# adam-kerrigan/pybader

Measured on AMD Instinct MI355X. Metric: Mvoxels/s neargrid assign+refine on 512^3 grid, higher is better.
Workload: dtype f64; 1 GPU; 512^3 synthetic 8-Gaussian-atom cubic cell (BASELINE config 3), neargrid assign + neargrid edge refinement changed:2, density resident in HBM; method=neargrid, device_driven_slab_step=False, basins=8

## Files before the change

### pybader_amd/csrc/host_assign.h

```cpp

static int read_counter(xb_ctx *c, int idx, int *out);
static GridL light(const Grid &g);

enum { BB_TOTAL = 1 << 20, BB_REGMAX = 1 << 16, BB_REGFIRST = 1 << 17 };

static bool table_windowed(const xb_ctx *c) { return c->g.wlen < c->g.nx; }

static int ensure_brick_bytes(xb_ctx *c, int nbr) {
    if (c->blab_alloc < nbr) {
        hipFree(c->blab_buf); c->blab_buf = nullptr; c->blab_alloc = 0; c->brick_rec = nullptr; c->brick_max_valid = false;
        if (c->grad_cover) { c->grad_cover = 0; c->grad_valid = false; }
        HIPCHK(hipMalloc(&c->blab_buf, (size_t)nbr * sizeof(int) + (size_t)nbr + 16));
        c->blab_alloc = nbr;
        c->brick_rec = reinterpret_cast<unsigned char *>(c->blab_buf + nbr);
    }
    return XB_OK;
}

static int ensure_grad(xb_ctx *c, bool force, bool boxes, bool main_rule) {
    if (int rc = need_grad(c)) return rc;
    c->g.main_ties = main_rule ? 1 : 0;
    if (c->grad_valid && !force && (c->grad_rule == 2 || c->grad_rule == (main_rule ? 1 : 0))) return XB_OK;
    const Grid &g = c->g;
    if (c->grad_valid && !force && !boxes && c->grad_cover == 1 && c->brick_rec) {
// ... 467 lines not shown
        else {
            k_buni_after_relabel<<<(nbr + 255) / 256, 256, 0, c->stream>>>(nbr, c->blab, box_max, c->first, buni, fs + FS_SORT_OK, nullptr, nullptr, nullptr);
            k_label_uniform_list<<<2048, TPB, 0, c->stream>>>(gl, c->labels, nb1, nb2, walk, 0, fs + FS_N_WALK, fs + FS_SORT_OK, buni);
        }
    } else
        k_relabel<<<nblocks(c->N), TPB, 0, c->stream>>>(g, c->labels, c->first, fs + FS_SORT_OK);
    k_reset_first<<<8, 256, 0, c->stream>>>(c->first, c->max_aux, 0, fs + FS_N_MAX, fs + FS_SORT_OK);
    HIPCHK(hipGetLastError());
    return XB_OK;
}

static int assign_neargrid_fused(xb_ctx *c, int64_t *n_maxima) {
    if (int rc = need_grad(c)) return rc;
    Grid &g = c->g;
    const GridL gl0 = light(g);
    const int nb0 = (g.nx + BRK - 1) / BRK, nb1 = (g.ny + BRK - 1) / BRK, nb2 = (g.nz + BRK - 1) / BRK, nbr = nb0 * nb1 * nb2;
    const bool part = g.nx % BRK || g.ny % BRK || g.nz % BRK;
    if (int rc = ensure_brick_bytes(c, nbr)) return rc;
    int *fs = c->fs;
    int *seed = c->list, *bmask = c->list + nbr, *buf0 = c->list + 2 * nbr, *buf1 = c->list + 3 * nbr, *walk = c->list + 4 * nbr;
    int *box_max = c->boxbuf + BB_REGMAX, *box_first = c->boxbuf + BB_REGFIRST;
    int *bmaxv = walk;
    int *bpot = c->list + 5 * nbr;
    const bool chase = true;
    int *bres = nullptr;
    c->box_max_tab = box_max;
    auto stage_done = [&](const char *what) {
        if (c->opt_dbg & 32) {
            const hipError_t e = (hipStreamSynchronize)(c->stream);
            int h16[16] = {0};
            (void)hipMemcpy(h16, fs, sizeof h16, hipMemcpyDeviceToHost);
            fprintf(stderr, "[assign] %s: %s  seeds %d regions %d certain %d walk %d maxima %d ovf %d err %d\n", what, hipGetErrorString(e), h16[FS_N_SEEDS],
                    h16[FS_N_BOXES], h16[FS_N_CERTAIN], h16[FS_N_WALK], h16[FS_N_MAX], h16[FS_N_OVF], h16[FS_ERR]);
            fflush(stderr);
        }
    };
    HIPCHK(hipMemsetAsync(fs, 0, FS_TOTAL * sizeof(int), c->stream));
    if (!c->first_clean) {
        k_fill<int><<<4096, TPB, 0, c->stream>>>(c->first, XB_INT_MAX, c->N);
        HIPCHK(hipGetLastError());
    }
    c->first_clean = false;
    c->regions_pending = false;
    c->buni_valid = false; c->regions_labels = false;
    c->list_valid = false; c->chg_n = -1;
    g.main_ties = 1;
    const GridL gl = light(g);
    (void)gl0;
    {
        ScopedTimer t4(c, 4);
        {
            ScopedTimer t5(c, 5);
            const int small = (g.nx < 16 || g.ny < 16 || g.nz < 80);
            dim3 grid((g.nz + GT_Z - 1) / GT_Z, (g.ny + GT_Y - 1) / GT_Y, (g.nx + GT_X - 1) / GT_X);
            GridS gs;
            const bool sym = sym_grid(g, gs);
            {
                int mirror = 0;
                double mu_scale = 0.;
                if (sym && c->opt_mirror) mirror_prefilter(g, mirror, mu_scale);
                const bool diag = c->opt_mask_diag && g.T[1] == 0. && g.T[2] == 0. && g.T[3] == 0. && g.T[5] == 0. && g.T[6] == 0. && g.T[7] == 0.;
                if (part) {
                    if (sym && diag) k_brick_masks<GridS, 1, true, true><<<grid, TPB, 0, c->stream>>>(gs, c->rho, small, bmask, bmaxv, fs + FS_TIES, 0, mu_scale, mirror, bpot);
                    else if (sym) k_brick_masks<GridS, 1, false, true><<<grid, TPB, 0, c->stream>>>(gs, c->rho, small, bmask, bmaxv, fs + FS_TIES, 0, mu_scale, mirror, bpot);
                    else k_brick_masks<Grid, 1, false, true><<<grid, TPB, 0, c->stream>>>(g, c->rho, small, bmask, bmaxv, fs + FS_TIES, 0, 0., 0, bpot);
                } else
                if (sym && diag) k_brick_masks<GridS, 1, true><<<grid, TPB, 0, c->stream>>>(gs, c->rho, small, bmask, bmaxv, fs + FS_TIES, 0, mu_scale, mirror, bpot);
                else if (sym) k_brick_masks<GridS, 1, false><<<grid, TPB, 0, c->stream>>>(gs, c->rho, small, bmask, bmaxv, fs + FS_TIES, 0, mu_scale, mirror, bpot);
                else k_brick_masks<Grid, 1, false><<<grid, TPB, 0, c->stream>>>(g, c->rho, small, bmask, bmaxv, fs + FS_TIES, 0, 0., 0, bpot);
            }
        }
        stage_done("brick masks");
        c->grad_valid = true;
        c->grad_rule = 1;
        c->grad_cover = 1;
        {
            k_seed_bricks<<<(nbr + 255) / 256, 256, 0, c->stream>>>(nbr, bmask, bmaxv, fs, seed, buf0, box_max, box_first);
            if (chase) {
                k_grow_parent<<<(nbr + TPB - 1) / TPB, TPB, 0, c->stream>>>(nb0, nb1, nb2, bmask, bpot, seed, buf1);
                k_grow_chase<<<(nbr + TPB - 1) / TPB, TPB, 0, c->stream>>>(nbr, buf1, seed, buf0, 4 * (nb0 + nb1 + nb2) + 64, fs);
            } else
                k_seed_finish<<<1, 1, 0, c->stream>>>(fs);
        }
        const int long_schedule = 2 * ((std::max(std::max(nb0, nb1), nb2) + BG - 1) / BG) + 12;
        const int launches = chase ? std::min(long_schedule, c->grow_kill_launches) : long_schedule;
        const dim3 ggrid((nb2 + BG - 1) / BG, (nb1 + BG - 1) / BG, (nb0 + BG - 1) / BG);
        for (int l = 0; l < launches; l++)
            k_brick_grow_dev<<<ggrid, BG * BG * BG, 0, c->stream>>>(nb0, nb1, nb2, bmask, seed, buf0, buf1, fs, BG, 0);
        k_grow_finish<<<64, TPB, 0, c->stream>>>(nbr, seed, buf0, buf1, fs, c->blab_buf, box_first, bmask, c->brick_rec, 0, chase && launches < long_schedule ? 1 : 0);
        HIPCHK(hipGetLastError());
        stage_done("region growth");
    }
    c->blab = c->blab_buf;
    c->regions_neargrid = true;
    c->walk = walk;
    c->nbk[0] = nb0; c->nbk[1] = nb1; c->nbk[2] = nb2;
    const long long own = c->N;
    {
        ScopedTimer t0(c, 0);
        {
            int bits = 0;
            while ((1 << bits) < std::max(std::max(nb0, nb1), nb2)) bits++;
            const unsigned n_codes = 1u << (3 * bits);
            const bool vac = c->has_vacuum && c->vac_by_tol;
            k_brick_walk_list_morton<<<(n_codes + 16 * TPB - 1) / (16 * TPB), TPB, 0, c->stream>>>(nb0, nb1, nb2, n_codes, c->blab, walk,
                                                                                                  fs + FS_N_WALK, fs + FS_GROW_RETRY,
                                                                                                  vac ? bpot : nullptr, c->vac_tol);
        }
        {
            ScopedTimer t7(c, 7);
            const int small = (g.nx < 16 || g.ny < 16 || g.nz < 80);
            GridS gs;
            if (sym_grid(g, gs))
                k_brick_records<GridS><<<4096, TPB, 0, c->stream>>>(gs, c->rho, c->grad, walk, fs + FS_N_WALK, nbr, nb1, nb2, c->brick_rec, small);
            else
                k_brick_records<Grid><<<4096, TPB, 0, c->stream>>>(g, c->rho, c->grad, walk, fs + FS_N_WALK, nbr, nb1, nb2, c->brick_rec, small);
        }
        stage_done("walk list + records");
        if (c->has_vacuum)
            k_fill_certain<<<nblocks(own), TPB, 0, c->stream>>>(gl, c->blab, nb1, nb2, box_max, c->labels, c->first, c->max_list,
                                                                fs + FS_N_MAX, c->max_cap, fs + FS_GROW_RETRY);
        else {
// ... 309 lines not shown
```

### pybader_amd/csrc/host_slab_table.h

```cpp


int xb_set_table_window(xb_ctx *c, int64_t margin) {
    NEED_GRID("xb_set_table_window");
    Grid &g = c->g;
    c->grad_valid = false;
    c->table_stage = 0;
    const int own = g.x1 - g.x0;
    if (margin < 0 || own == g.nx) { g.wx0 = 0; g.wlen = g.nx; c->table_margin = -1; g.wbase = 0; return XB_OK; }
    if (g.nx % 8 || g.ny % 8 || g.nz % 8 || g.x0 % 8 || g.x1 % 8)
        return fail(XB_E_ARG, "xb_set_table_window: grid and slab must be made of whole 8^3 bricks");
    const int m8 = (int)((std::max<int64_t>(margin, c->halo) + 7) / 8) * 8;
    if (own + 2 * m8 >= g.nx) { g.wx0 = 0; g.wlen = g.nx; c->table_margin = -1; g.wbase = 0; return XB_OK; }
    g.wx0 = ((g.x0 - m8) % g.nx + g.nx) % g.nx;
    g.wlen = own + 2 * m8;
    c->table_margin = m8;
    return need_grad(c);
}
static bool slab_sparse_ok(const xb_ctx *c) {
    const Grid &g = c->g;
    return c->opt_boxes && c->opt_bricks && table_windowed(c) && g.nx % BRK == 0 && g.ny % BRK == 0 && g.nz % BRK == 0 &&
           g.x0 % BRK == 0 && g.x1 % BRK == 0 && g.ny >= 16 && g.nz >= 16 && 7LL * (c->N / (BRK * BRK * BRK)) <= c->N;
}
int xb_table_build(xb_ctx *c, int64_t *n_local_seeds) {
    NEED_GRID_RAW("xb_table_build");
    if (int rc = need_grad(c)) return rc;
    c->slab_sparse = false;
    if (slab_sparse_ok(c)) {
        Grid &g = c->g;
        const int nb1 = g.ny / BRK, nb2 = g.nz / BRK, nbr = (g.nx / BRK) * nb1 * nb2;
        if (int rc = ensure_brick_bytes(c, nbr)) return rc;
        int *fs = c->fs, *bmask = c->list + nbr, *bmaxv = c->list + 4 * nbr;
        HIPCHK(hipMemsetAsync(fs, 0, FS_TOTAL * sizeof(int), c->stream));
        g.main_ties = 1;
        {
            ScopedTimer t4(c, 4);
            ScopedTimer t5(c, 5);
            const int small = (g.nx < 16 || g.ny < 16 || g.nz < 80);
            dim3 grid((g.nz + GT_Z - 1) / GT_Z, (g.ny + GT_Y - 1) / GT_Y, (g.x1 - g.x0) / GT_X);
            GridS gs;
            int mirror = 0;
            double mu_scale = 0.;
            if (c->opt_mirror) mirror_prefilter(g, mirror, mu_scale);
            if (sym_grid(g, gs)) k_brick_masks<GridS, 1, false><<<grid, TPB, 0, c->stream>>>(gs, c->rho, small, bmask, bmaxv, fs + FS_TIES, g.x0, mu_scale, mirror, nullptr);
            else k_brick_masks<Grid, 1, false><<<grid, TPB, 0, c->stream>>>(g, c->rho, small, bmask, bmaxv, fs + FS_TIES, g.x0, 0., 0, nullptr);
        }
        HIPCHK(hipGetLastError());
        int ties = 0;
        HIPCHK(hipMemcpyAsync(c->host_ints, fs + FS_TIES, sizeof(int), hipMemcpyDeviceToHost, c->stream));
        HIPCHK(hipStreamSynchronize(c->stream));
        ties = c->host_ints[0];
        c->window_ties = ties != 0;
        c->window_seeds.clear();
        c->grad_valid = true;
        c->grad_cover = 1;
        c->grad_rule = 1;
        c->blab = nullptr;
        c->n_boxes = 0; c->box_voxels = 0;
        c->table_stage = 1;
        c->slab_sparse = true;
        if (n_local_seeds) *n_local_seeds = 0;
        return XB_OK;
    }
    if (int rc = ensure_grad(c, true, true, true)) return rc;
    if (n_local_seeds) *n_local_seeds = table_windowed(c) ? (int64_t)c->window_seeds.size() : 0;
    return XB_OK;
}
int xb_table_local_seeds(xb_ctx *c, int64_t *out, int64_t capacity) {
    NEED_GRID_RAW("xb_table_local_seeds");
    if ((int64_t)c->window_seeds.size() > capacity) return fail(XB_E_ARG, "xb_table_local_seeds: capacity too small");
    for (size_t i = 0; i < c->window_seeds.size(); i++) out[i] = c->window_seeds[i];
    return XB_OK;
}
int xb_brick_masks(xb_ctx *c, void **dev_ptr, int64_t *n_bricks, int64_t *own_first, int64_t *own_count) {
    NEED_GRID_RAW("xb_brick_masks");
    const Grid &g = c->g;
    if (g.nx % 8 || g.ny % 8 || g.nz % 8) return fail(XB_E_STATE, "xb_brick_masks: grid is not made of whole bricks");
    const int64_t nbr = c->N / 512, per_plane = (int64_t)(g.ny / 8) * (g.nz / 8);
    if (dev_ptr) *dev_ptr = (void *)(c->list + nbr);
    if (n_bricks) *n_bricks = nbr;
    if (own_first) *own_first = (g.x0 / 8) * per_plane;
    if (own_count) *own_count = ((g.x1 - g.x0) / 8) * per_plane;
    return XB_OK;
}
int xb_table_ties(xb_ctx *c, int64_t *has_ties) {
    NEED_GRID_RAW("xb_table_ties");
    if (c->table_stage < 1 || !c->grad_valid) return fail(XB_E_STATE, "xb_table_ties: call xb_table_build first");
    if (has_ties) *has_ties = c->window_ties ? 1 : 0;
    return XB_OK;
}
int xb_table_finish(xb_ctx *c, const int64_t *seeds, int64_t n_seeds, int64_t any_ties) {
    NEED_GRID_RAW("xb_table_finish");
    if (c->table_stage < 1 || !c->grad_valid) return fail(XB_E_STATE, "xb_table_finish: call xb_table_build first");
    c->grad_rule = any_ties ? 1 : 2;
    if (c->slab_sparse) {
        Grid &g = c->g;
        const GridL gl = light(g);
        const int nb0 = g.nx / BRK, nb1 = g.ny / BRK, nb2 = g.nz / BRK, nbr = nb0 * nb1 * nb2;
// ... 100 lines not shown
```

### pybader_amd/csrc/k_masks.h

```cpp
#pragma once

#define GT_X 8
#define GT_Y 8
#define GT_Z 32

#define BRK 8
#define BG 8

__device__ __forceinline__ int wrap_any(int v, int n) { v %= n; return v < 0 ? v + n : v; }

__global__ void k_flag_window_bricks(int nb0, int per_plane, int b0, int nb, unsigned char flag, unsigned char *brick_rec) {
    const int b = blockIdx.x * blockDim.x + threadIdx.x;
    if (b >= nb0 * per_plane) return;
    int d = b / per_plane - b0;
    if (d < 0) d += nb0;
    brick_rec[b] = d < nb ? flag : (unsigned char)0;
}


#define BM_EPS 2e-12
#ifdef XB_DEBUG_COUNT
__device__ unsigned long long xb_dbg[65536];
__device__ signed char *xb_dbg_steps;
#endif
// ... 183 lines not shown
                                         int x0, int y0, int z0, int mirror) {
    {
        const int wv = __builtin_amdgcn_readfirstlane(threadIdx.x / XB_WAVE), lane = threadIdx.x % XB_WAVE;
        const int lz = min(lane, GT_Z + 1);
        int Z = z0 + lz - 1;
        unsigned Yw[GT_Y + 2];
        Z = SMALL ? ((Z % g.nz) + g.nz) % g.nz : wrap_u(Z, g.nz);
        const unsigned zoff = (unsigned)Z * 8u;
#pragma unroll
        for (int ey = 0; ey < GT_Y + 2; ey++) {
            int Y = y0 + ey - 1;
            if (SMALL) Y = ((Y % g.ny) + g.ny) % g.ny;
            else if (PART || ey == 0 || ey == GT_Y + 1) Y = wrap_u(Y, g.ny);
            Yw[ey] = (unsigned)(Y * g.nz) * 8u;
        }
        constexpr int PL = (GT_X + 2 + 3) / 4;
        double val[PL][GT_Y + 2];
#pragma unroll
        for (int j = 0; j < PL; j++) {
            const int ex = wv + 4 * j;
            if (ex < GT_X + 2) {
                int X = x0 + ex - 1;
                X = SMALL ? ((X % g.nx) + g.nx) % g.nx : wrap_u(X, g.nx);
                const char *plane = reinterpret_cast<const char *>(rho + (size_t)X * g.nyz);
#pragma unroll
                for (int ey = 0; ey < GT_Y + 2; ey++) val[j][ey] = *reinterpret_cast<const double *>(plane + Yw[ey] + zoff);
            } else {
#pragma unroll
                for (int ey = 0; ey < GT_Y + 2; ey++) val[j][ey] = 0.;
            }
        }
        if (lane < GT_Z + 2) {
#pragma unroll
            for (int j = 0; j < PL; j++) {
                const int ex = wv + 4 * j;
                if (ex < GT_X + 2) {
#pragma unroll
                    for (int ey = 0; ey < GT_Y + 2; ey++) tile[ex][ey][lane] = val[j][ey];
                }
            }
        }
        if (mirror) {
            unsigned hi = 0;
#pragma unroll
            for (int j = 0; j < PL; j++)
#pragma unroll
                for (int ey = 0; ey < GT_Y + 2; ey++) hi = max(hi, (unsigned)__double2hiint(val[j][ey]) & 0x7fffffffu);
#pragma unroll
            for (int o = 32; o > 0; o >>= 1) hi = max(hi, (unsigned)__shfl_xor((int)hi, o));
            if (lane == 0) atomicMax(s_bmax, hi);
        }
    }
}
template <typename GT, int MT, bool DIAG, bool PART = false>
__global__ __launch_bounds__(TPB) void k_brick_masks(GT g, const double *__restrict__ rho, int small, int *__restrict__ bmask,
                                                     int *__restrict__ bmaxv, int *tie_count, int xbase, double mu_scale, int mirror,
                                                     int *__restrict__ bpot) {
    __shared__ double tile[GT_X + 2][GT_Y + 2][BM_ROW];
    __shared__ int s_mask[GT_Z / 8], s_cnt[GT_Z / 8], s_mv[GT_Z / 8], s_pot[GT_Z / 8];
    __shared__ unsigned s_bmax;
    const int x0 = xbase + blockIdx.z * GT_X, y0 = blockIdx.y * GT_Y, z0 = blockIdx.x * GT_Z;
    if (threadIdx.x < GT_Z / 8) { s_mask[threadIdx.x] = 0; s_cnt[threadIdx.x] = 0; s_mv[threadIdx.x] = -1; s_pot[threadIdx.x] = -2147483647 - 1; }
    if (threadIdx.x == 0) s_bmax = 0;
    __syncthreads();
    if (small & 1) bm_stage<true, PART>(g, rho, tile, &s_bmax, x0, y0, z0, mirror);
    else bm_stage<false, PART>(g, rho, tile, &s_bmax, x0, y0, z0, mirror);
    __syncthreads();
    const double mu = mirror ? __hiloint2double((int)min(s_bmax + 1u, 0x7ff00000u), 0) * mu_scale : 0.;
    int ty, tz;
    bm_column(threadIdx.x, ty, tz);
    const int zz = tz & 7;
    const int wx = PART ? min(GT_X, g.nx - x0) : GT_X, wy = PART ? min(8, g.ny - y0) : 8, wz = PART ? min(8, g.nz - (z0 + (tz & ~7))) : 8;
    const bool at_yh = ty == wy - 1, at_zh = zz == wz - 1;
    const bool deep = __builtin_amdgcn_readfirstlane(threadIdx.x / XB_WAVE) == 3 && (!PART || (wx == GT_X && wy == 8 && z0 + GT_Z <= g.nz));
    const double kInf = __builtin_huge_val();
    BmCoef co;
    co.yl = ty == 0 ? BM_EPS : (ty == 1 ? -(1. - BM_EPS) : -kInf);
    co.yh = at_yh ? -BM_EPS : (ty == wy - 2 ? (1. - BM_EPS) : kInf);
    co.zl = zz == 0 ? BM_EPS : (zz == 1 ? -(1. - BM_EPS) : -kInf);
    co.zh = at_zh ? -BM_EPS : (zz == wz - 2 ? (1. - BM_EPS) : kInf);
    const int y = y0 + ty, z = z0 + tz;
    const bool col_in = y < g.ny && z < g.nz;
    const double dface = fmin(fmin(fmin(dist_at(g, 0, 1, 1), dist_at(g, 2, 1, 1)), fmin(dist_at(g, 1, 0, 1), dist_at(g, 1, 2, 1))),
                              fmin(dist_at(g, 1, 1, 0), dist_at(g, 1, 1, 2)));
    double a[3][3][3];
#pragma unroll
    for (int iy = 0; iy < 3; iy++)
#pragma unroll
        for (int iz = 0; iz < 3; iz++) {
            a[1][iy][iz] = tile[0][ty + iy][tz + iz];
            a[2][iy][iz] = tile[1][ty + iy][tz + iz];
        }
    int mine = 0;
    bool any_tie = false;
    double cmax = -1.7976931348623157e308;
#define BM_STEP(K)                                                                                                   \
    {                                                                                                                \
        _Pragma("unroll") for (int iy = 0; iy < 3; iy++) _Pragma("unroll") for (int iz = 0; iz < 3; iz++) {          \
            a[0][iy][iz] = a[1][iy][iz];                                                                             \
            a[1][iy][iz] = a[2][iy][iz];                                                                             \
            a[2][iy][iz] = tile[K + 2][ty + iy][tz + iz];                                                            \
        }                                                                                                            \
        const int x = x0 + K;                                                                                        \
        if (!PART || x < g.nx) cmax = max_raw(cmax, a[1][1][1]);    \
        bm_voxel<MT, K, DIAG, PART>(g, a, dface, col_in && x < g.nx, (x * g.ny + y) * g.nz + z, ty, zz, mine, any_tie, \
                                    &s_cnt[tz >> 3], &s_mv[tz >> 3], mu, mirror, co, deep, wx, at_yh, at_zh);          \
    }
    BM_STEP(0) BM_STEP(1) BM_STEP(2) BM_STEP(3) BM_STEP(4) BM_STEP(5) BM_STEP(6) BM_STEP(7)
#undef BM_STEP
    static_assert(GT_X == 8, "eight x-positions per column");
    if (__any(any_tie) && threadIdx.x % XB_WAVE == 0) atomicAdd(tie_count, 1);
    atomicOr(&s_mask[tz >> 3], mine);
    if (bpot && col_in) {
        const int fi = __float_as_int((float)cmax);
        atomicMax(&s_pot[tz >> 3], fi >= 0 ? fi : fi ^ 0x7fffffff);
    }
    __syncthreads();
    if (threadIdx.x < GT_Z / 8 && z0 + threadIdx.x * 8 < g.nz) {
        const int nb1 = (g.ny + 7) >> 3, nb2 = (g.nz + 7) >> 3;
        if (bpot) bpot[((x0 >> 3) * nb1 + (y0 >> 3)) * nb2 + (z0 >> 3) + threadIdx.x] = s_pot[threadIdx.x];
        const int b = ((x0 >> 3) * nb1 + (y0 >> 3)) * nb2 + (z0 >> 3) + threadIdx.x, n = s_cnt[threadIdx.x];
        const bool dead = PART && (g.nx - x0 == 1 || g.ny - y0 == 1 || g.nz - (z0 + 8 * (int)threadIdx.x) == 1);
        bmask[b] = (s_mask[threadIdx.x] & 0x7ffdfff) | ((n >= 1 || dead) ? 1 << 27 : 0) | ((n >= 2 || dead) ? 1 << 28 : 0);
        bmaxv[b] = (n == 1 && !dead) ? s_mv[threadIdx.x] : -1;
    }
}

#define BR_ROW 24
template <typename GT>
__global__ __launch_bounds__(TPB, 4) void k_brick_records(GT g, const double *__restrict__ rho, GradRec *__restrict__ G,
                                                       const int *__restrict__ walk, const int *n_list, int nbr, int nb1, int nb2,
                                                       unsigned char *brick_rec, int small) {
    __shared__ double tile[10][10][BR_ROW];
    const int n = walk ? *n_list : nbr;
    int goff[4], loff[4];
#pragma unroll
    for (int j = 0; j < 4; j++) {
        const int e = threadIdx.x + j * TPB;
        const int ex = e / 100, ey = (e / 10) % 10, ez = e % 10;
        goff[j] = (ex * g.ny + ey) * g.nz + ez;
        loff[j] = (ex * 10 + ey) * BR_ROW + ez;
    }
    const XcdRange xr = xcd_range(n);
    for (int item = xr.begin; item < xr.end; item += xr.step) {
        const int b = walk ? walk[item] : item;
        if (!walk && !(brick_rec[b] & 1)) continue;
        const int b0 = b / (nb1 * nb2), b1 = (b / nb2) % nb1, b2 = b % nb2;
        const int x0 = b0 * 8, y0 = b1 * 8, z0 = b2 * 8;
        const bool inner = !(small & 1) && x0 >= 1 && x0 + 8 < g.nx && y0 >= 1 && y0 + 8 < g.ny && z0 >= 1 && z0 + 8 < g.nz;
        __syncthreads();
        {
            double val[4];
            if (inner) {
                const double *corner = rho + ((size_t)(x0 - 1) * g.ny + (y0 - 1)) * g.nz + (z0 - 1);
#pragma unroll
                for (int j = 0; j < 4; j++) val[j] = (threadIdx.x + j * TPB < 1000) ? corner[goff[j]] : 0.;
            } else {
#pragma unroll
                for (int j = 0; j < 4; j++) {
                    const int e = threadIdx.x + j * TPB;
                    const int ex = e / 100, ey = (e / 10) % 10, ez = e % 10;
                    int X = x0 + ex - 1, Y = y0 + ey - 1, Z = z0 + ez - 1;
                    if (small & 1) {
                        X = ((X % g.nx) + g.nx) % g.nx; Y = ((Y % g.ny) + g.ny) % g.ny; Z = ((Z % g.nz) + g.nz) % g.nz;
                    } else {
                        X = wrap_u(X, g.nx); Y = wrap_u(Y, g.ny); Z = wrap_u(Z, g.nz);
                    }
                    val[j] = e < 1000 ? rho[(X * g.ny + Y) * g.nz + Z] : 0.;
                }
            }
#pragma unroll
            for (int j = 0; j < 4; j++)
                if (threadIdx.x + j * TPB < 1000) (&tile[0][0][0])[loff[j]] = val[j];
        }
        __syncthreads();
        const int vbase = (x0 * g.ny + y0) * g.nz + z0;
#pragma unroll 1
        for (int j = 0; j < 2; j++) {
// ... 87 lines not shown
```

### pybader_amd/csrc/slab_step.h

```cpp

#define XB_TAB_ROWS 1024
#define XB_TAB_INTS (2 + 2 * XB_TAB_ROWS)
#define XB_SLAB_RANKS_MAX 64
#define XB_XCNT 8
__host__ __device__ __forceinline__ size_t walk_part(int cap) { return 16 + (size_t)cap * (sizeof(Walker) + 8); }
static inline int walk_cap_for(const Grid &g) { return (int)std::min<long long>(std::max<long long>(32768, (long long)g.nyz / 8), 1 << 20); }

__global__ void k_slab_flag(const int *fs, int *flags, int rank) { flags[rank] = fs[FS_TIES] != 0; }
__global__ void k_slab_any_flag(const int *flags, int nranks, int *fs) {
    int any = 0;
    for (int r = 0; r < nranks; r++) any |= flags[r];
    fs[FS_TIES] = any;
}
__global__ void k_slab_pack_table(int *tab, const int *__restrict__ max_list, const int *__restrict__ first, int *fs,
                                  const int *slow_count) {
    const int n = fs[FS_N_MAX];
    const bool bad = n > XB_TAB_ROWS || *slow_count > 0 || fs[FS_GROW_RETRY];
    if (threadIdx.x == 0) { tab[0] = bad ? -1 : n; tab[1] = 0; fs[FS_N_REDO] = fs[FS_N_OVF]; fs[FS_N_OVF] = *slow_count; }
    if (bad) return;
    for (int i = threadIdx.x; i < n; i += blockDim.x) {
        const int m = max_list[i];
        tab[2 + 2 * i] = m;
        tab[3 + 2 * i] = first[m];
    }
// ... 93 lines not shown
static int slab_need_wbuf(xb_ctx *c) {
    const int n = std::max(c->slab_nranks, 1), cap = walk_cap_for(c->g);
    if (c->wbuf[0] && c->wbuf_ranks >= n && c->wcap == cap) return XB_OK;
    HIPCHK(hipStreamSynchronize(c->stream));
    for (int k = 0; k < 2; k++) { (void)hipFree(c->wbuf[k]); c->wbuf[k] = nullptr; }
    (void)hipFree(c->wk_in); c->wk_in = nullptr;
    for (int k = 0; k < 2; k++) {
        HIPCHK(hipMalloc(&c->wbuf[k], (size_t)n * walk_part(cap)));
        HIPCHK(hipMemsetAsync(c->wbuf[k], 0, (size_t)n * walk_part(cap), c->stream));
    }
    HIPCHK(hipMalloc(&c->wk_in, (size_t)cap * sizeof(Walker) + 16));
    c->wbuf_ranks = n;
    c->wcap = cap;
    return XB_OK;
}

static bool slab_step_ok(const xb_ctx *c, int nranks) {
    const Grid &g = c->g;
    const long long nbr = c->N / (BRK * BRK * BRK);
    return slab_sparse_ok(c) && !c->has_vacuum && nranks >= 2 && nranks <= XB_SLAB_RANKS_MAX && g.nz % 4 == 0 &&
           c->list_cap >= 7 * nbr && c->halo >= 3;
}

extern "C" {

int xb_host_waits(int64_t *n) {
    if (n) *n = xb_waits;
    return XB_OK;
}

int xb_slab_supported(xb_ctx *c, int nranks, int64_t *ok) {
    NEED_GRID_RAW("xb_slab_supported");
    if (ok) *ok = slab_step_ok(c, nranks) ? 1 : 0;
    return XB_OK;
}

int xb_slab_assign_masks(xb_ctx *c, int rank, int nranks) {
    NEED_GRID_RAW("xb_slab_assign_masks");
    if (rank < 0 || rank >= nranks) return fail(XB_E_ARG, "xb_slab_assign_masks: bad rank");
    if (!slab_step_ok(c, nranks)) return fail(XB_E_STATE, "xb_slab_assign_masks: this slab cannot take the device-driven step (see xb_slab_supported)");
    if (int rc = need_grad(c)) return rc;
    if (int rc = slab_need_xbuf(c)) return rc;
    Grid &g = c->g;
    const int nb1 = g.ny / BRK, nb2 = g.nz / BRK, nbr = (g.nx / BRK) * nb1 * nb2;
    if (int rc = ensure_brick_bytes(c, nbr)) return rc;
    c->slab_rank = rank; c->slab_nranks = nranks;
    int *fs = c->fs, *bmask = c->list + nbr, *bmaxv = c->list + 4 * nbr, *bpot = c->list + 5 * nbr;
    HIPCHK(hipMemsetAsync(fs, 0, FS_TOTAL * sizeof(int), c->stream));
    g.main_ties = 1;
    {
        ScopedTimer t4(c, 4);
        ScopedTimer t5(c, 5);
        const int small = (g.nx < 16 || g.ny < 16 || g.nz < 80);
        dim3 grid((g.nz + GT_Z - 1) / GT_Z, (g.ny + GT_Y - 1) / GT_Y, (g.x1 - g.x0) / GT_X);
        GridS gs;
        int mirror = 0;
        double mu_scale = 0.;
        const bool sym = sym_grid(g, gs);
        if (sym && c->opt_mirror) mirror_prefilter(g, mirror, mu_scale);
        const bool diag = c->opt_mask_diag && g.T[1] == 0. && g.T[2] == 0. && g.T[3] == 0. && g.T[5] == 0. && g.T[6] == 0. && g.T[7] == 0.;
        if (sym && diag) k_brick_masks<GridS, 1, true><<<grid, TPB, 0, c->stream>>>(gs, c->rho, small, bmask, bmaxv, fs + FS_TIES, g.x0, mu_scale, mirror, bpot);
        else if (sym) k_brick_masks<GridS, 1, false><<<grid, TPB, 0, c->stream>>>(gs, c->rho, small, bmask, bmaxv, fs + FS_TIES, g.x0, mu_scale, mirror, bpot);
        else k_brick_masks<Grid, 1, false><<<grid, TPB, 0, c->stream>>>(g, c->rho, small, bmask, bmaxv, fs + FS_TIES, g.x0, 0., 0, bpot);
        k_slab_flag<<<1, 1, 0, c->stream>>>(fs, slab_flags(c), rank);
    }
    HIPCHK(hipGetLastError());
    c->slab_sparse = true;
    c->window_seeds.clear();
    c->grad_valid = true;
    c->grad_cover = 1;
    c->grad_rule = 1;
    c->blab = nullptr;
    c->n_boxes = 0; c->box_voxels = 0;
    c->table_stage = 1;
    c->slab_stage = 1;
    return XB_OK;
}

int xb_slab_block(xb_ctx *c, int which, void **dev_ptr, int64_t *bytes_total, int64_t *own_offset, int64_t *own_bytes) {
    NEED_GRID_RAW("xb_slab_block");
    if (!c->xbuf || c->slab_nranks < 1) return fail(XB_E_STATE, "xb_slab_block: call xb_slab_assign_masks first");
    const Grid &g = c->g;
    const int64_t nbr = c->N / 512, per_plane = (int64_t)(g.ny / 8) * (g.nz / 8);
    void *p = nullptr;
    int64_t total = 0, off = 0, own = 0;
    if (which >= 0 && which <= 2) {
        p = c->list + (which == 0 ? nbr : (which == 1 ? 4 * nbr : 5 * nbr));
        total = nbr * 4; off = (g.x0 / 8) * per_plane * 4; own = ((g.x1 - g.x0) / 8) * per_plane * 4;
    } else if (which == 3) { p = slab_flags(c); total = c->slab_nranks * 4; off = c->slab_rank * 4; own = 4; }
    else if (which == 4) { p = slab_tables(c); total = (int64_t)c->slab_nranks * XB_TAB_INTS * 4; off = (int64_t)c->slab_rank * XB_TAB_INTS * 4; own = XB_TAB_INTS * 4; }
    else if (which == 5) { p = slab_counts(c); total = 2 * XB_XCNT * 8; off = 0; own = XB_XCNT * 8; }
    else if (which == 6 || which == 7) {
        if (int rc = slab_need_wbuf(c)) return rc;
        p = c->wbuf[which - 6]; total = (int64_t)c->slab_nranks * walk_part(c->wcap); off = (int64_t)c->slab_rank * walk_part(c->wcap); own = walk_part(c->wcap);
    }
    else return fail(XB_E_ARG, "xb_slab_block: unknown block %d", which);
    if (dev_ptr) *dev_ptr = p;
    if (bytes_total) *bytes_total = total;
    if (own_offset) *own_offset = off;
    if (own_bytes) *own_bytes = own;
    return XB_OK;
}
static inline int walk_send_of(const xb_ctx *c, int cap) { return c->walk_send > 0 ? std::min(c->walk_send, cap) : cap; }
static inline int walk_later_of(const xb_ctx *c, int cap) { return std::min(cap / 8, walk_send_of(c, cap)); }
static inline int walk_results_of(const xb_ctx *c, int cap) {
    return (int)std::min<long long>(cap, (long long)walk_send_of(c, cap) * std::max(c->slab_nranks, 1));
}
int xb_slab_walk_send(xb_ctx *c, int64_t walkers) {
    NEED_GRID_RAW("xb_slab_walk_send");
    c->walk_send = walkers <= 0 ? 0 : (int)std::min<int64_t>(std::max<int64_t>(walkers, 1024), 1 << 20);
    return XB_OK;
}
int xb_slab_walk_layout(xb_ctx *c, int64_t out[5]) {
    NEED_GRID_RAW("xb_slab_walk_layout");
    if (!out) return fail(XB_E_ARG, "xb_slab_walk_layout: null argument");
    const int cap = walk_cap_for(c->g);
// ... 320 lines not shown
```

Baseline: 42190 Mvoxels/s.

## Make brick-mask kernel persistent along x with async LDS-staged plane ring buffer

Each workgroup now walks a run of bricks along x instead of handling one 8-plane brick. Halo planes are reused between consecutive bricks, and rho planes are prefetched into a three-slot LDS ring with buffer_load_lds while the current planes are being processed. Runs are remapped so work is spread across the XCDs, and the mirror plane-max is computed per plane from LDS. The aim is to cut redundant halo reads and to hide global load latency in the brick-mask pass. In exchange the grid holds fewer workgroups, the kernel needs more explicit barriers, and it relies on AMD-specific intrinsics.

```diff
diff --git a/pybader_amd/csrc/host_assign.h b/pybader_amd/csrc/host_assign.h
--- a/pybader_amd/csrc/host_assign.h
+++ b/pybader_amd/csrc/host_assign.h
@@ -543,7 +543,8 @@
         {
             ScopedTimer t5(c, 5);
             const int small = (g.nx < 16 || g.ny < 16 || g.nz < 80);
-            dim3 grid((g.nz + GT_Z - 1) / GT_Z, (g.ny + GT_Y - 1) / GT_Y, (g.nx + GT_X - 1) / GT_X);
+            int run_bricks, n_runs;
+            bm_runs(nb0, g.ny, g.nz, run_bricks, n_runs);
             GridS gs;
             const bool sym = sym_grid(g, gs);
             {
@@ -552,13 +553,13 @@
                 if (sym && c->opt_mirror) mirror_prefilter(g, mirror, mu_scale);
                 const bool diag = c->opt_mask_diag && g.T[1] == 0. && g.T[2] == 0. && g.T[3] == 0. && g.T[5] == 0. && g.T[6] == 0. && g.T[7] == 0.;
                 if (part) {
-                    if (sym && diag) k_brick_masks<GridS, 1, true, true><<<grid, TPB, 0, c->stream>>>(gs, c->rho, small, bmask, bmaxv, fs + FS_TIES, 0, mu_scale, mirror, bpot);
-                    else if (sym) k_brick_masks<GridS, 1, false, true><<<grid, TPB, 0, c->stream>>>(gs, c->rho, small, bmask, bmaxv, fs + FS_TIES, 0, mu_scale, mirror, bpot);
-                    else k_brick_masks<Grid, 1, false, true><<<grid, TPB, 0, c->stream>>>(g, c->rho, small, bmask, bmaxv, fs + FS_TIES, 0, 0., 0, bpot);
+                    if (sym && diag) k_brick_masks<GridS, 1, true, true><<<n_runs, TPB, 0, c->stream>>>(gs, c->rho, small, bmask, bmaxv, fs + FS_TIES, 0, nb0, run_bricks, mu_scale, mirror, bpot);
+                    else if (sym) k_brick_masks<GridS, 1, false, true><<<n_runs, TPB, 0, c->stream>>>(gs, c->rho, small, bmask, bmaxv, fs + FS_TIES, 0, nb0, run_bricks, mu_scale, mirror, bpot);
+                    else k_brick_masks<Grid, 1, false, true><<<n_runs, TPB, 0, c->stream>>>(g, c->rho, small, bmask, bmaxv, fs + FS_TIES, 0, nb0, run_bricks, 0., 0, bpot);
                 } else
-                if (sym && diag) k_brick_masks<GridS, 1, true><<<grid, TPB, 0, c->stream>>>(gs, c->rho, small, bmask, bmaxv, fs + FS_TIES, 0, mu_scale, mirror, bpot);
-                else if (sym) k_brick_masks<GridS, 1, false><<<grid, TPB, 0, c->stream>>>(gs, c->rho, small, bmask, bmaxv, fs + FS_TIES, 0, mu_scale, mirror, bpot);
-                else k_brick_masks<Grid, 1, false><<<grid, TPB, 0, c->stream>>>(g, c->rho, small, bmask, bmaxv, fs + FS_TIES, 0, 0., 0, bpot);
+                if (sym && diag) k_brick_masks<GridS, 1, true><<<n_runs, TPB, 0, c->stream>>>(gs, c->rho, small, bmask, bmaxv, fs + FS_TIES, 0, nb0, run_bricks, mu_scale, mirror, bpot);
+                else if (sym) k_brick_masks<GridS, 1, false><<<n_runs, TPB, 0, c->stream>>>(gs, c->rho, small, bmask, bmaxv, fs + FS_TIES, 0, nb0, run_bricks, mu_scale, mirror, bpot);
+                else k_brick_masks<Grid, 1, false><<<n_runs, TPB, 0, c->stream>>>(g, c->rho, small, bmask, bmaxv, fs + FS_TIES, 0, nb0, run_bricks, 0., 0, bpot);
             }
         }
         stage_done("brick masks");
diff --git a/pybader_amd/csrc/host_slab_table.h b/pybader_amd/csrc/host_slab_table.h
--- a/pybader_amd/csrc/host_slab_table.h
+++ b/pybader_amd/csrc/host_slab_table.h
@@ -36,13 +36,14 @@
             ScopedTimer t4(c, 4);
             ScopedTimer t5(c, 5);
             const int small = (g.nx < 16 || g.ny < 16 || g.nz < 80);
-            dim3 grid((g.nz + GT_Z - 1) / GT_Z, (g.ny + GT_Y - 1) / GT_Y, (g.x1 - g.x0) / GT_X);
+            int run_bricks, n_runs;
+            bm_runs((g.x1 - g.x0) / GT_X, g.ny, g.nz, run_bricks, n_runs);
             GridS gs;
             int mirror = 0;
             double mu_scale = 0.;
             if (c->opt_mirror) mirror_prefilter(g, mirror, mu_scale);
-            if (sym_grid(g, gs)) k_brick_masks<GridS, 1, false><<<grid, TPB, 0, c->stream>>>(gs, c->rho, small, bmask, bmaxv, fs + FS_TIES, g.x0, mu_scale, mirror, nullptr);
-            else k_brick_masks<Grid, 1, false><<<grid, TPB, 0, c->stream>>>(g, c->rho, small, bmask, bmaxv, fs + FS_TIES, g.x0, 0., 0, nullptr);
+            if (sym_grid(g, gs)) k_brick_masks<GridS, 1, false><<<n_runs, TPB, 0, c->stream>>>(gs, c->rho, small, bmask, bmaxv, fs + FS_TIES, g.x0, (g.x1 - g.x0) / GT_X, run_bricks, mu_scale, mirror, nullptr);
+            else k_brick_masks<Grid, 1, false><<<n_runs, TPB, 0, c->stream>>>(g, c->rho, small, bmask, bmaxv, fs + FS_TIES, g.x0, (g.x1 - g.x0) / GT_X, run_bricks, 0., 0, nullptr);
         }
         HIPCHK(hipGetLastError());
         int ties = 0;
diff --git a/pybader_amd/csrc/k_masks.h b/pybader_amd/csrc/k_masks.h
--- a/pybader_amd/csrc/k_masks.h
+++ b/pybader_amd/csrc/k_masks.h
@@ -259,27 +259,108 @@
         }
     }
 }
+#define BM_PL 352
+#define BM_PIECES 11
+#define BM_GRP 4
+#define BM_SLOT (BM_GRP * BM_PL)
+#define BM_NSLOT 3
+#define BM_MIN_WG 2048
+static_assert((GT_Y + 2) * BM_ROW <= BM_PL && BM_PL * 2 == BM_PIECES * 64, "a plane is 11 pieces of 64 dwords");
+
+static inline void bm_runs(int nbx, int ny, int nz, int &run_bricks, int &n_runs) {
+    const int faces = ((ny + GT_Y - 1) / GT_Y) * ((nz + GT_Z - 1) / GT_Z);
+    int nxr = std::min(nbx, std::max(1, (BM_MIN_WG + faces - 1) / faces));
+    run_bricks = (nbx + nxr - 1) / nxr;
+    nxr = (nbx + run_bricks - 1) / run_bricks;
+    n_runs = nxr * faces;
+}
+
+__device__ __forceinline__ void bm_barrier() {
+    asm volatile("s_waitcnt lgkmcnt(0)" ::: "memory");
+    __builtin_amdgcn_s_barrier();
+    asm volatile("" ::: "memory");
+}
+template <typename GT>
+__device__ __forceinline__ void bm_fill(const GT &g, const double *__restrict__ rho, double *dst, int xp, int p0, int small,
+                                        const unsigned *s_off, int wv) {
+    unsigned off[3];
+#pragma unroll
+    for (int k = 0; k < 3; k++) off[k] = s_off[k * TPB + threadIdx.x];
+    for (int p = p0; p < BM_GRP; p++) {
+        int X = xp + p;
+        X = small ? ((X % g.nx) + g.nx) % g.nx : wrap_u(X, g.nx);
+        const __amdgpu_buffer_rsrc_t plane = __builtin_amdgcn_make_buffer_rsrc((void *)(rho + (size_t)X * g.nyz), (short)0, -1, 0x00020000);
+#pragma unroll
+        for (int k = 0; k < 3; k++) {
+            const int j = wv + 4 * k;
+            if (j < BM_PIECES)
+                __builtin_amdgcn_raw_ptr_buffer_load_lds(plane, (__attribute__((address_space(3))) void *)(dst + p * BM_PL + 32 * j), 4,
+                                                         off[k], 0, 0, 0);
+        }
+    }
+}
+template <typename GT>
+__device__ __forceinline__ void bm_offsets(const GT &g, int y0, int z0, int small, int wv, int lane, unsigned *s_off) {
+#pragma unroll
+    for (int k = 0; k < 3; k++) {
+        const int e = 64 * (wv + 4 * k) + lane;
+        int row = GT_Y + 1, col = GT_Z + 1;
+        if (e < (GT_Y + 2) * BM_ROW * 2) {
+            row = e / (2 * BM_ROW);
+            col = min((e - 2 * BM_ROW * row) >> 1, GT_Z + 1);
+        }
+        int Y = y0 + row - 1, Z = z0 + col - 1;
+        if (small) { Y = ((Y % g.ny) + g.ny) % g.ny; Z = ((Z % g.nz) + g.nz) % g.nz; }
+        else { Y = wrap_u(Y, g.ny); Z = wrap_u(Z, g.nz); }
+        s_off[k * TPB + threadIdx.x] = ((unsigned)(Y * g.nz) + (unsigned)Z) * 8u + 4u * (unsigned)(e & 1);
+    }
+}
+__device__ __forceinline__ unsigned bm_plane_max(const double *pl, int lane) {
+    const unsigned *w = reinterpret_cast<const unsigned *>(pl);
+    unsigned hi = 0;
+#pragma unroll
+    for (int k = 0; k < 6; k++) {
+        const int i = lane + 64 * k;
+        if (i < BM_PL) hi = max(hi, w[2 * i + 1] & 0x7fffffffu);
+    }
+#pragma unroll
+    for (int o = 32; o > 0; o >>= 1) hi = max(hi, (unsigned)__shfl_xor((int)hi, o));
+    return hi;
+}
+
 template <typename GT, int MT, bool DIAG, bool PART = false>
 __global__ __launch_bounds__(TPB) void k_brick_masks(GT g, const double *__restrict__ rho, int small, int *__restrict__ bmask,
-                                                     int *__restrict__ bmaxv, int *tie_count, int xbase, double mu_scale, int mirror,
-                                                     int *__restrict__ bpot) {
-    __shared__ double tile[GT_X + 2][GT_Y + 2][BM_ROW];
-    __shared__ int s_mask[GT_Z / 8], s_cnt[GT_Z / 8], s_mv[GT_Z / 8], s_pot[GT_Z / 8];
-    __shared__ unsigned s_bmax;
-    const int x0 = xbase + blockIdx.z * GT_X, y0 = blockIdx.y * GT_Y, z0 = blockIdx.x * GT_Z;
-    if (threadIdx.x < GT_Z / 8) { s_mask[threadIdx.x] = 0; s_cnt[threadIdx.x] = 0; s_mv[threadIdx.x] = -1; s_pot[threadIdx.x] = -2147483647 - 1; }
-    if (threadIdx.x == 0) s_bmax = 0;
-    __syncthreads();
-    if (small & 1) bm_stage<true, PART>(g, rho, tile, &s_bmax, x0, y0, z0, mirror);
-    else bm_stage<false, PART>(g, rho, tile, &s_bmax, x0, y0, z0, mirror);
-    __syncthreads();
-    const double mu = mirror ? __hiloint2double((int)min(s_bmax + 1u, 0x7ff00000u), 0) * mu_scale : 0.;
+                                                     int *__restrict__ bmaxv, int *tie_count, int xbase, int nbx, int run_bricks,
+                                                     double mu_scale, int mirror, int *__restrict__ bpot) {
+    __shared__ double lds[BM_NSLOT * BM_SLOT + 16 + 3 * TPB / 2];
+    int *const s_mask = reinterpret_cast<int *>(lds + BM_NSLOT * BM_SLOT), *const s_cnt = s_mask + 4, *const s_mv = s_mask + 8,
+              *const s_pot = s_mask + 12;
+    unsigned *const s_pmax = reinterpret_cast<unsigned *>(s_mask + 16), *const s_off = s_pmax + 16;
+    static_assert(GT_Z / 8 == 4, "four bricks per face row");
+    const int nty = (g.ny + GT_Y - 1) / GT_Y, ntz = (g.nz + GT_Z - 1) / GT_Z;
+    const int nwg = (int)gridDim.x, xcd = (int)blockIdx.x % 8, q8 = nwg / 8, r8 = nwg % 8;
+    const int run = (xcd < r8 ? xcd * (q8 + 1) : r8 * (q8 + 1) + (xcd - r8) * q8) + (int)blockIdx.x / 8;
+    const int y0 = ((run / ntz) % nty) * GT_Y, z0 = (run % ntz) * GT_Z;
+    const int bx0 = (run / (ntz * nty)) * run_bricks, nb = min(run_bricks, nbx - bx0);
+    const int X0 = xbase + bx0 * GT_X;
+    const int wv = __builtin_amdgcn_readfirstlane(threadIdx.x / XB_WAVE), lane = threadIdx.x % XB_WAVE;
     int ty, tz;
     bm_column(threadIdx.x, ty, tz);
+    bm_offsets(g, y0, z0, small, wv, lane, s_off);
+    bm_fill(g, rho, lds + 2 * BM_SLOT, X0 - 3, 2, small, s_off, wv);
+    bm_fill(g, rho, lds, X0 + 1, 0, small, s_off, wv);
+    bm_fill(g, rho, lds + BM_SLOT, X0 + 5, 0, small, s_off, wv);
+    if (threadIdx.x < GT_Z / 8) { s_mask[threadIdx.x] = 0; s_cnt[threadIdx.x] = 0; s_mv[threadIdx.x] = -1; s_pot[threadIdx.x] = -2147483647 - 1; }
+    asm volatile("s_waitcnt vmcnt(0)" ::: "memory");
+    bm_barrier();
+    if (mirror) {
+        if (wv >= 2) { const unsigned h = bm_plane_max(lds + 2 * BM_SLOT + wv * BM_PL, lane); if (lane == 0) s_pmax[wv - 2] = h; }
+        const unsigned h0 = bm_plane_max(lds + wv * BM_PL, lane), h1 = bm_plane_max(lds + BM_SLOT + wv * BM_PL, lane);
+        if (lane == 0) { s_pmax[2 + wv] = h0; s_pmax[6 + wv] = h1; }
+    }
     const int zz = tz & 7;
-    const int wx = PART ? min(GT_X, g.nx - x0) : GT_X, wy = PART ? min(8, g.ny - y0) : 8, wz = PART ? min(8, g.nz - (z0 + (tz & ~7))) : 8;
+    const int wy = PART ? min(8, g.ny - y0) : 8, wz = PART ? min(8, g.nz - (z0 + (tz & ~7))) : 8;
     const bool at_yh = ty == wy - 1, at_zh = zz == wz - 1;
-    const bool deep = __builtin_amdgcn_readfirstlane(threadIdx.x / XB_WAVE) == 3 && (!PART || (wx == GT_X && wy == 8 && z0 + GT_Z <= g.nz));
     const double kInf = __builtin_huge_val();
     BmCoef co;
     co.yl = ty == 0 ? BM_EPS : (ty == 1 ? -(1. - BM_EPS) : -kInf);
@@ -291,46 +372,85 @@
     const double dface = fmin(fmin(fmin(dist_at(g, 0, 1, 1), dist_at(g, 2, 1, 1)), fmin(dist_at(g, 1, 0, 1), dist_at(g, 1, 2, 1))),
                               fmin(dist_at(g, 1, 1, 0), dist_at(g, 1, 1, 2)));
     double a[3][3][3];
+    const int lofs = ty * BM_ROW + tz;
 #pragma unroll
     for (int iy = 0; iy < 3; iy++)
 #pragma unroll
         for (int iz = 0; iz < 3; iz++) {
-            a[1][iy][iz] = tile[0][ty + iy][tz + iz];
-            a[2][iy][iz] = tile[1][ty + iy][tz + iz];
-        }
-    int mine = 0;
+            a[1][iy][iz] = lds[2 * BM_SLOT + 2 * BM_PL + lofs + iy * BM_ROW + iz];
+            a[2][iy][iz] = lds[2 * BM_SLOT + 3 * BM_PL + lofs + iy * BM_ROW + iz];
+        }
+    bm_barrier();
     bool any_tie = false;
-    double cmax = -1.7976931348623157e308;
+    auto flush = [&](int x0) {
+        if (threadIdx.x < GT_Z / 8) {
+            if (z0 + threadIdx.x * 8 < g.nz) {
+                const int nb1 = (g.ny + 7) >> 3, nb2 = (g.nz + 7) >> 3;
+                const int b = ((x0 >> 3) * nb1 + (y0 >> 3)) * nb2 + (z0 >> 3) + threadIdx.x, n = s_cnt[threadIdx.x];
+                if (bpot) bpot[b] = s_pot[threadIdx.x];
+                const bool dead = PART && (g.nx - x0 == 1 || g.ny - y0 == 1 || g.nz - (z0 + 8 * (int)threadIdx.x) == 1);
+                bmask[b] = (s_mask[threadIdx.x] & 0x7ffdfff) | ((n >= 1 || dead) ? 1 << 27 : 0) | ((n >= 2 || dead) ? 1 << 28 : 0);
+                bmaxv[b] = (n == 1 && !dead) ? s_mv[threadIdx.x] : -1;
+            }
+            s_mask[threadIdx.x] = 0; s_cnt[threadIdx.x] = 0; s_mv[threadIdx.x] = -1; s_pot[threadIdx.x] = -2147483647 - 1;
+        }
+    };
+#pragma unroll 1
+    for (int i = 0; i < nb; i++) {
+        const int x0 = X0 + i * GT_X;
+        if (i > 0) {
+            asm volatile("s_waitcnt vmcnt(0)" ::: "memory");
+            bm_barrier();
+            flush(x0 - GT_X);
+            if (mirror) {
+                const unsigned h0 = bm_plane_max(lds + ((2 * i) % 3) * BM_SLOT + wv * BM_PL, lane);
+                const unsigned h1 = bm_plane_max(lds + ((2 * i + 1) % 3) * BM_SLOT + wv * BM_PL, lane);
+                if (lane == 0) { s_pmax[(8 * i + 2 + wv) & 15] = h0; s_pmax[(8 * i + 6 + wv) & 15] = h1; }
+            }
+        }
+        if (i + 1 < nb) bm_fill(g, rho, lds + ((2 * i + 2) % 3) * BM_SLOT, X0 + 8 * i + 9, 0, small, s_off, wv);
+        bm_barrier();
+        double mu = 0.;
+        if (mirror) {
+            unsigned hi = 0;
+#pragma unroll
+            for (int k = 0; k < GT_X + 2; k++) hi = max(hi, s_pmax[(8 * i + k) & 15]);
+            hi = __builtin_amdgcn_readfirstlane(hi);
+            mu = __hiloint2double((int)min(hi + 1u, 0x7ff00000u), 0) * mu_scale;
+        }
+        const int wx = PART ? min(GT_X, g.nx - x0) : GT_X;
+        const bool deep = wv == 3 && (!PART || (wx == GT_X && wy == 8 && z0 + GT_Z <= g.nz));
+        int mine = 0;
+        double cmax = -1.7976931348623157e308;
+        const double *pl = lds + ((2 * i) % 3) * BM_SLOT + lofs;
 #define BM_STEP(K)                                                                                                   \
     {                                                                                                                \
         _Pragma("unroll") for (int iy = 0; iy < 3; iy++) _Pragma("unroll") for (int iz = 0; iz < 3; iz++) {          \
             a[0][iy][iz] = a[1][iy][iz];                                                                             \
             a[1][iy][iz] = a[2][iy][iz];                                                                             \
-            a[2][iy][iz] = tile[K + 2][ty + iy][tz + iz];                                                            \
+            a[2][iy][iz] = pl[((K) % BM_GRP) * BM_PL + iy * BM_ROW + iz];                                            \
         }                                                                                                            \
         const int x = x0 + K;                                                                                        \
         if (!PART || x < g.nx) cmax = max_raw(cmax, a[1][1][1]);    \
         bm_voxel<MT, K, DIAG, PART>(g, a, dface, col_in && x < g.nx, (x * g.ny + y) * g.nz + z, ty, zz, mine, any_tie, \
                                     &s_cnt[tz >> 3], &s_mv[tz >> 3], mu, mirror, co, deep, wx, at_yh, at_zh);          \
     }
-    BM_STEP(0) BM_STEP(1) BM_STEP(2) BM_STEP(3) BM_STEP(4) BM_STEP(5) BM_STEP(6) BM_STEP(7)
+        BM_STEP(0) BM_STEP(1) BM_STEP(2) BM_STEP(3)
+        bm_barrier();
+        if (i + 1 < nb) bm_fill(g, rho, lds + ((2 * i) % 3) * BM_SLOT, X0 + 8 * i + 13, 0, small, s_off, wv);
+        pl = lds + ((2 * i + 1) % 3) * BM_SLOT + lofs;
+        BM_STEP(4) BM_STEP(5) BM_STEP(6) BM_STEP(7)
 #undef BM_STEP
-    static_assert(GT_X == 8, "eight x-positions per column");
-    if (__any(any_tie) && threadIdx.x % XB_WAVE == 0) atomicAdd(tie_count, 1);
-    atomicOr(&s_mask[tz >> 3], mine);
-    if (bpot && col_in) {
-        const int fi = __float_as_int((float)cmax);
-        atomicMax(&s_pot[tz >> 3], fi >= 0 ? fi : fi ^ 0x7fffffff);
-    }
-    __syncthreads();
-    if (threadIdx.x < GT_Z / 8 && z0 + threadIdx.x * 8 < g.nz) {
-        const int nb1 = (g.ny + 7) >> 3, nb2 = (g.nz + 7) >> 3;
-        if (bpot) bpot[((x0 >> 3) * nb1 + (y0 >> 3)) * nb2 + (z0 >> 3) + threadIdx.x] = s_pot[threadIdx.x];
-        const int b = ((x0 >> 3) * nb1 + (y0 >> 3)) * nb2 + (z0 >> 3) + threadIdx.x, n = s_cnt[threadIdx.x];
-        const bool dead = PART && (g.nx - x0 == 1 || g.ny - y0 == 1 || g.nz - (z0 + 8 * (int)threadIdx.x) == 1);
-        bmask[b] = (s_mask[threadIdx.x] & 0x7ffdfff) | ((n >= 1 || dead) ? 1 << 27 : 0) | ((n >= 2 || dead) ? 1 << 28 : 0);
-        bmaxv[b] = (n == 1 && !dead) ? s_mv[threadIdx.x] : -1;
-    }
+        static_assert(GT_X == 8, "eight x-positions per column");
+        atomicOr(&s_mask[tz >> 3], mine);
+        if (bpot && col_in) {
+            const int fi = __float_as_int((float)cmax);
+            atomicMax(&s_pot[tz >> 3], fi >= 0 ? fi : fi ^ 0x7fffffff);
+        }
+    }
+    bm_barrier();
+    flush(X0 + (nb - 1) * GT_X);
+    if (__any(any_tie) && lane == 0) atomicAdd(tie_count, 1);
 }
 
 #define BR_ROW 24
diff --git a/pybader_amd/csrc/slab_step.h b/pybader_amd/csrc/slab_step.h
--- a/pybader_amd/csrc/slab_step.h
+++ b/pybader_amd/csrc/slab_step.h
@@ -169,16 +169,17 @@
         ScopedTimer t4(c, 4);
         ScopedTimer t5(c, 5);
         const int small = (g.nx < 16 || g.ny < 16 || g.nz < 80);
-        dim3 grid((g.nz + GT_Z - 1) / GT_Z, (g.ny + GT_Y - 1) / GT_Y, (g.x1 - g.x0) / GT_X);
+        int run_bricks, n_runs;
+        bm_runs((g.x1 - g.x0) / GT_X, g.ny, g.nz, run_bricks, n_runs);
         GridS gs;
         int mirror = 0;
         double mu_scale = 0.;
         const bool sym = sym_grid(g, gs);
         if (sym && c->opt_mirror) mirror_prefilter(g, mirror, mu_scale);
         const bool diag = c->opt_mask_diag && g.T[1] == 0. && g.T[2] == 0. && g.T[3] == 0. && g.T[5] == 0. && g.T[6] == 0. && g.T[7] == 0.;
-        if (sym && diag) k_brick_masks<GridS, 1, true><<<grid, TPB, 0, c->stream>>>(gs, c->rho, small, bmask, bmaxv, fs + FS_TIES, g.x0, mu_scale, mirror, bpot);
-        else if (sym) k_brick_masks<GridS, 1, false><<<grid, TPB, 0, c->stream>>>(gs, c->rho, small, bmask, bmaxv, fs + FS_TIES, g.x0, mu_scale, mirror, bpot);
-        else k_brick_masks<Grid, 1, false><<<grid, TPB, 0, c->stream>>>(g, c->rho, small, bmask, bmaxv, fs + FS_TIES, g.x0, 0., 0, bpot);
+        if (sym && diag) k_brick_masks<GridS, 1, true><<<n_runs, TPB, 0, c->stream>>>(gs, c->rho, small, bmask, bmaxv, fs + FS_TIES, g.x0, (g.x1 - g.x0) / GT_X, run_bricks, mu_scale, mirror, bpot);
+        else if (sym) k_brick_masks<GridS, 1, false><<<n_runs, TPB, 0, c->stream>>>(gs, c->rho, small, bmask, bmaxv, fs + FS_TIES, g.x0, (g.x1 - g.x0) / GT_X, run_bricks, mu_scale, mirror, bpot);
+        else k_brick_masks<Grid, 1, false><<<n_runs, TPB, 0, c->stream>>>(g, c->rho, small, bmask, bmaxv, fs + FS_TIES, g.x0, (g.x1 - g.x0) / GT_X, run_bricks, 0., 0, bpot);
         k_slab_flag<<<1, 1, 0, c->stream>>>(fs, slab_flags(c), rank);
     }
     HIPCHK(hipGetLastError());
```

Result: slower. 39250 Mvoxels/s, median of 2 (-7.0%).
